# neptune-ai/open-solution-mapping-challenge

Hardware: NVIDIA H100
Metric: 300x300 tiles/sec fwd+bwd ResNet101-UNet (higher is better)
Workload: dtype bf16

## Files before the change

### include/mcb200.h

```cpp
#ifndef MCB200_H_
#define MCB200_H_

#include <stddef.h>
#include <stdint.h>

#ifdef __cplusplus
extern "C" {
#endif

#define MCB_OK 0
#define MCB_ERR_INVALID (-1)
#define MCB_ERR_CUDA (-2)
#define MCB_ERR_UNSUPPORTED (-3)

const char* mcb_last_error(void);
int mcb_version(void);
int mcb_zero_bytes(void* p, size_t bytes, void* stream);


typedef struct {
  const void* x[2];
  int cin[2];
  int n, h, w;
  const void* weight;
// ... 44 lines not shown
typedef struct {
  const void* x;
  int n, h, w, cin;
  const void* weight;
  int cout;
  const float* bias;
  int relu;
  void* y;
  int ksize;
} mcb_convt_fwd_args;
int mcb_convt_fwd(const mcb_convt_fwd_args* a, void* stream);

typedef struct {
  const void* dy;
  int n, h, w, cin;
  const void* weight;
  int cout;
  void* dx;
  const void* relu_mask;
  int accumulate;
  float* dx_channel_sum;
  int ksize;
} mcb_convt_dgrad_args;
int mcb_convt_dgrad(const mcb_convt_dgrad_args* a, void* stream);

typedef struct {
  const void* dy;
  const void* x;
  int n, h, w, cin, cout;
  float* dw;
  int ksize;
} mcb_convt_wgrad_args;
int mcb_convt_wgrad(const mcb_convt_wgrad_args* a, void* stream);


int mcb_nchw_f32_to_nhwc_bf16(const float* x, void* y, int n, int c, int h, int w, void* stream);
int mcb_nhwc_bf16_to_nchw_f32(const void* x, float* y, int n, int c, int h, int w, void* stream);

int mcb_stem_im2col(const float* x_nchw, void* col, int n, int h, int w, void* stream);
int mcb_stem_pack_weight(const float* w, void* w_packed, void* stream);
int mcb_stem_unpack_wgrad(const float* dw_packed, float* dw, void* stream);

int mcb_vgg_input_im2col(const float* x_nchw, void* col, int n, int h, int w, void* stream);
int mcb_vgg_input_pack_weight(const float* w, void* w_packed, void* stream);
int mcb_vgg_input_unpack_wgrad(const float* dw_packed, float* dw, void* stream);

int mcb_bn_finalize(const float* stats, long count, const float* gamma, const float* beta, float* running_mean,
                    float* running_var, float momentum, float eps, float* scale, float* shift, float* mean,
                    float* invstd, int c, void* stream);
int mcb_bn_eval_params(const float* gamma, const float* beta, const float* running_mean, const float* running_var,
                       float eps, float* scale, float* shift, int c, void* stream);
int mcb_bn_apply(const void* z, const float* scale, const float* shift, const void* residual, const float* res_scale,
                 const float* res_shift, int relu, void* y, long pixels, int c, void* stream);
typedef struct {
  const float* stats;
  const float* gamma;
  const float* beta;
  float* running_mean;
  float* running_var;
  float* mean;
  float* invstd;
} mcb_bn_train;
int mcb_bn_train_apply(const void* z, const mcb_bn_train* bn, const void* residual, const mcb_bn_train* res_bn, int relu,
                       void* y, long pixels, int c, float momentum, float eps, void* stream);
int mcb_bn_train_apply_global(const void* z, const mcb_bn_train* bn, const void* residual, const mcb_bn_train* res_bn,
                              int relu, void* y, long pixels, long stat_count, int c, float momentum, float eps,
// ... 164 lines not shown
```

### open-solution-mapping-challenge_b200/_lib.py

```python
import ctypes as C
import os

_HERE = os.path.dirname(os.path.abspath(__file__))
LIB_PATH = os.path.join(_HERE, "libmcb200.so")

if not os.path.exists(LIB_PATH):
    raise ImportError(
        "libmcb200.so not built: run `python __graft_entry__.py` (nvcc, sm_90a). There is no CPU fallback.")

lib = C.CDLL(LIB_PATH)
lib.mcb_last_error.restype = C.c_char_p
lib.mcb_version.restype = C.c_int

vp, ci, fp = C.c_void_p, C.c_int, C.POINTER(C.c_float)


class ConvFwdArgs(C.Structure):
    _fields_ = [("x", vp * 2), ("cin", ci * 2), ("n", ci), ("h", ci), ("w", ci), ("weight", vp), ("cout", ci),
                ("ksize", ci), ("stride", ci), ("bias", vp), ("relu", ci), ("stats", vp), ("y", vp), ("scale", vp),
                ("residual", vp)]


class ConvDgradArgs(C.Structure):
    _fields_ = [("dy", vp), ("n", ci), ("h", ci), ("w", ci), ("weight", vp), ("cout", ci), ("cin_total", ci),
                ("ci_off", ci), ("cin", ci), ("ksize", ci), ("stride", ci), ("dx", vp), ("relu_mask", vp),
                ("accumulate", ci), ("bn_z", vp), ("bn_mean", vp), ("bn_invstd", vp), ("bn_dbeta", vp),
                ("bn_dgamma", vp), ("bn_gamma", vp), ("bn_beta", vp), ("dx_channel_sum", vp)]


class ConvWgradArgs(C.Structure):
    _fields_ = [("dy", vp), ("x", vp), ("n", ci), ("h", ci), ("w", ci), ("cout", ci), ("cin_total", ci),
                ("ci_off", ci), ("cin", ci), ("ksize", ci), ("stride", ci), ("dw", vp)]


class ConvtFwdArgs(C.Structure):
    _fields_ = [("x", vp), ("n", ci), ("h", ci), ("w", ci), ("cin", ci), ("weight", vp), ("cout", ci), ("bias", vp),
                ("relu", ci), ("y", vp), ("ksize", ci)]


class ConvtDgradArgs(C.Structure):
    _fields_ = [("dy", vp), ("n", ci), ("h", ci), ("w", ci), ("cin", ci), ("weight", vp), ("cout", ci), ("dx", vp),
                ("relu_mask", vp), ("accumulate", ci), ("dx_channel_sum", vp), ("ksize", ci)]


class ConvtWgradArgs(C.Structure):
    _fields_ = [("dy", vp), ("x", vp), ("n", ci), ("h", ci), ("w", ci), ("cin", ci), ("cout", ci), ("dw", vp),
                ("ksize", ci)]


def check(rc, what=""):
    if rc != 0:
        raise RuntimeError("libmcb200 %s failed (%d): %s" % (what, rc, lib.mcb_last_error().decode()))


def ptr(t):
    return None if t is None else C.c_void_p(t.data_ptr())


def stream_ptr():
    import torch
    return C.c_void_p(torch.cuda.current_stream().cuda_stream)


def call(name, args=None, *extra):
    fn = getattr(lib, name)
    if args is None:
        rc = fn(*extra, stream_ptr())
    else:
        rc = fn(C.byref(args), *extra, stream_ptr())
    check(rc, name)


class LossArgs(C.Structure):
    _fields_ = [("logits", vp), ("target", vp), ("n", ci), ("h", ci), ("w", ci), ("mode", ci), ("w0", C.c_float),
                ("sigma", C.c_float), ("size_c", C.c_float), ("dice_weight", C.c_float), ("ce_weight", C.c_float),
                ("dice_smooth", C.c_float), ("dice_activation", ci)]


cl, cf = C.c_long, C.c_float
_SIGS = {
    "mcb_nchw_f32_to_nhwc_bf16": [vp, vp, ci, ci, ci, ci, vp],
    "mcb_nhwc_bf16_to_nchw_f32": [vp, vp, ci, ci, ci, ci, vp],
    "mcb_stem_im2col": [vp, vp, ci, ci, ci, vp],
    "mcb_stem_pack_weight": [vp, vp, vp],
    "mcb_stem_unpack_wgrad": [vp, vp, vp],
    "mcb_vgg_input_im2col": [vp, vp, ci, ci, ci, vp],
    "mcb_vgg_input_pack_weight": [vp, vp, vp],
    "mcb_vgg_input_unpack_wgrad": [vp, vp, vp],
    "mcb_maxpool2_bwd_skip_relu": [vp, vp, vp, vp, ci, ci, ci, ci, vp],
    "mcb_bn_finalize": [vp, cl, vp, vp, vp, vp, cf, cf, vp, vp, vp, vp, ci, vp],
    "mcb_bn_eval_params": [vp, vp, vp, vp, cf, vp, vp, ci, vp],
    "mcb_bn_apply": [vp, vp, vp, vp, vp, vp, ci, vp, cl, ci, vp],
    "mcb_bn_bwd_reduce": [vp, vp, vp, vp, vp, vp, vp, cl, ci, vp],
    "mcb_bn_bwd_apply": [vp, vp, vp, vp, vp, vp, vp, vp, vp, vp, ci, cl, ci, vp],
    "mcb_bn_bwd_apply_global": [vp, vp, vp, vp, vp, vp, vp, vp, vp, vp, ci, cl, cl, ci, vp],
    "mcb_channel_sum": [vp, vp, cl, ci, vp],
    "mcb_det_sum_f32": [vp, ci, cl, cl, cl, vp, cl, vp],
    "mcb_maxpool2_fwd": [vp, vp, ci, ci, ci, ci, vp],
    "mcb_maxpool2_bwd": [vp, vp, vp, ci, ci, ci, ci, ci, vp],
    "mcb_final_conv_fwd": [vp, vp, vp, vp, ci, ci, ci, ci, ci, vp],
    "mcb_final_conv_bwd": [vp, vp, vp, vp, vp, vp, ci, ci, ci, ci, ci, vp],
    "mcb_adam_step": [vp, vp, vp, vp, vp, cl, cf, C.c_double, C.c_double, cf, cf, ci, cf, vp],
    "mcb_adam_step_dyn": [vp, vp, vp, vp, vp, cl, vp, cf, cf, cf, cf, cf, vp],
    "mcb_cast_f32_bf16": [vp, vp, cl, vp],
    "mcb_loss_partials": [C.POINTER(LossArgs), vp, vp],
    "mcb_loss_grad": [C.POINTER(LossArgs), vp, cl, cf, vp, vp, vp],
    "mcb_softmax2": [vp, vp, ci, ci, ci, vp],
}
for _n, _a in _SIGS.items():
    getattr(lib, _n).argtypes = _a
    getattr(lib, _n).restype = ci
for _n in ("mcb_conv_fwd", "mcb_conv_dgrad", "mcb_conv_wgrad", "mcb_convt_fwd", "mcb_convt_dgrad", "mcb_convt_wgrad"):
    getattr(lib, _n).restype = ci


def dp(t):
    return None if t is None else t.data_ptr()


def fcall(name, *args):
    import torch
    rc = getattr(lib, name)(*args, torch.cuda.current_stream().cuda_stream)
    check(rc, name)

_SIGS2 = {
    "mcb_resize_bilinear_f64": [vp, vp, vp, ci, ci, ci, ci, ci, ci, vp],
    "mcb_threshold_layers": [vp, ci, vp, vp, vp, ci, ci, ci, ci, ci, vp],
    "mcb_ccl_label": [vp, ci, vp, vp, vp, ci, ci, ci, vp],
    "mcb_morph_rect": [vp, vp, ci, ci, ci, ci, ci, ci, vp],
    "mcb_add_dropped_objects": [vp, vp, vp, vp, ci, ci, ci, vp],
    "mcb_instance_scores": [vp, vp, ci, vp, vp, vp, vp, ci, ci, ci, ci, vp],
}
for _n, _a in _SIGS2.items():
    getattr(lib, _n).argtypes = _a
    getattr(lib, _n).restype = ci

_SIGS3 = {
    "mcb_crf_rgb_from_normalized": [vp, vp, ci, ci, ci, vp],
    "mcb_dense_crf": [vp, vp, vp, vp, ci, ci, ci, cf, cf, cf, cf, cf, ci, vp],
}
for _n, _a in _SIGS3.items():
    getattr(lib, _n).argtypes = _a
    getattr(lib, _n).restype = ci

lib.mcb_watershed.argtypes = [vp, ci, vp, vp, vp, vp, ci, ci, ci, ci, vp]
lib.mcb_watershed.restype = ci
# ... 94 lines not shown
```

### open-solution-mapping-challenge_b200/csrc/conv_gemm.cu

```cuda
#include "host_common.h"
#include "conv_gemm.cuh"
#include "../../include/mcb200.h"
#include <algorithm>
#include <mutex>
#include <stdlib.h>

namespace mcb {

static void pick_tile(int Wv, int Hv, int N, int max_rows, int row_mult, int* pbw, int* pbh, int* pbn) {
  double best = -1.0;
  int bbw = 1, bbh = 1, bbn = 1;
  for (int bw = 1; bw <= std::min(max_rows, std::min(Wv, 256)); ++bw) {
    for (int bh = 1; bw * bh <= max_rows && bh <= std::min(Hv, 256); ++bh) {
      const int bn_max = std::min(256, max_rows / (bw * bh));
      for (int bn = 1; bn <= bn_max; ++bn) {
        if (bn > N && row_mult == 1) break;
        const int rows = bw * bh * bn;
        if (rows % row_mult != 0) continue;
        const long tiles = (long)((Wv + bw - 1) / bw) * ((Hv + bh - 1) / bh) * ((N + bn - 1) / bn);
        const double eff = (double)Wv * Hv * N / ((double)tiles * max_rows);
        const double score = eff + 1e-6 * bw + 1e-9 * bh;
        if (score > best) {
          best = score;
          bbw = bw; bbh = bh; bbn = bn;
        }
      }
    }
  }
  *pbw = bbw; *pbh = bbh; *pbn = bbn;
}

constexpr int kSmemBudget = 227 * 1024;
constexpr int kMaxStagesHalo = 9, kMaxStages = 6;
constexpr int kWgradMaxStages = 8;
constexpr int kTwoStagingMinStages = 3;
constexpr int kHaloMinChannels = 128;
constexpr int kBn256MinWaveX10 = 6;
constexpr int kWgradWavesX10 = 10;
constexpr int kWgradMinKb = 6;
constexpr int kWgradKbTarget = 64;
constexpr int kWgradMinWaveX10 = 4;

static_assert(conv_smem(32, 32, true, kMaxStagesHalo, 1, 0).fits && conv_smem(32, 32, false, kMaxStages, 1, 0).fits &&
                  wgrad_smem(32, kWgradMaxStages).fits, "the mbarriers outgrow their reserve at the deepest rings");

struct TestHooks { int force_bn, halo, wgrad_splits; };
static TestHooks test_hooks() {
  auto get = [](const char* name, int dflt) {
    const char* v = getenv(name);
    return v ? atoi(v) : dflt;
  };
  return {get("MCB_FORCE_BN", 0), get("MCB_HALO", 2), get("MCB_WGRAD_SPLITS", 0)};
}

template <auto Kernel, class Params>
static int launch_kernel(const Params& p, dim3 grid, int threads, size_t smem, cudaStream_t st) {
  static bool attr_set = false;
  if (!attr_set) {
    MCB_CHECK_CUDA(cudaFuncSetAttribute(Kernel, cudaFuncAttributeMaxDynamicSharedMemorySize, kSmemBudget));
    attr_set = true;
  }
  Kernel<<<grid, threads, smem, st>>>(p);
  MCB_LAUNCH_CHECK();
  return MCB_OK;
}

static int launch_conv_kernel(int BN, int BK, bool b_mn, bool halo, const ConvGemmParams& p, dim3 grid, size_t smem,
                              cudaStream_t st) {
  auto with_flag = [](bool v, auto f) { return v ? f(std::true_type()) : f(std::false_type()); };
  return with_flag(BK == 64, [&](auto bk64) { return with_flag(b_mn, [&](auto mn) { return with_flag(halo, [&](auto h) {
    constexpr int K = decltype(bk64)::value ? 64 : 32;
    constexpr bool M = decltype(mn)::value, H = decltype(h)::value;
    switch (BN) {
      case 256: return launch_kernel<conv_gemm_kernel<256, K, M, H>>(p, grid, kConvThreads, smem, st);
      case 128: return launch_kernel<conv_gemm_kernel<128, K, M, H>>(p, grid, kConvThreads, smem, st);
      case 64: return launch_kernel<conv_gemm_kernel<64, K, M, H>>(p, grid, kConvThreads, smem, st);
      case 32: return launch_kernel<conv_gemm_kernel<32, K, M, H>>(p, grid, kConvThreads, smem, st);
    }
    return fail(MCB_ERR_UNSUPPORTED, "unsupported BN %d", BN);
  }); }); });
}

static int launch_conv(int BN, int BK, bool b_mn, ConvGemmParams& p, int m_tiles, int n_tiles, int phases,
                       cudaStream_t st, bool halo = false) {
  auto layout = [&](int stages, int out_bufs) { return conv_smem(BN, BK, halo, stages, out_bufs, p.aux_mode != 0); };
  const int stage = layout(0, 0).stage, max_stages = halo ? kMaxStagesHalo : kMaxStages;
  p.out_bufs = (kSmemBudget - layout(0, 2).bytes) / stage >= kTwoStagingMinStages ? 2 : 1;
  p.stages = std::max(2, std::min(max_stages, (kSmemBudget - layout(0, p.out_bufs).bytes) / stage));
  p.m_tiles = m_tiles; p.n_tiles = n_tiles; p.phases = phases;
  const size_t smem = layout(p.stages, p.out_bufs).bytes;
  const long total = (long)m_tiles * n_tiles * phases;
  dim3 grid((unsigned)std::min<long>(total, num_sms()), 1, 1);
  const int nch = n_tiles * BN;
  const bool red = conv_reduces(p);
  p.red_stride = 2 * nch;
  if (red && (long)grid.x * p.red_stride > kConvRedCap)
    return fail(MCB_ERR_UNSUPPORTED, "conv: reduction rows %u x %d exceed the workspace", grid.x, p.red_stride);
  const int r = launch_conv_kernel(BN, BK, b_mn, halo, p, grid, smem, st);
  if (r || !red) return r;
  const int rows = (int)grid.x;
  if (p.aux_mode == 0) {
    conv_red_finish_kernel<<<det_finish_grid(2L * nch, rows), kDetFinishThreads, 0, st>>>(
        0L, rows, (long)p.red_stride, 2L * nch, (long)nch, p.stats + p.n_off, (long)p.stats_c);
  } else {
    conv_red_finish_kernel<<<det_finish_grid(nch, rows), kDetFinishThreads, 0, st>>>(
        0L, rows, (long)p.red_stride, (long)nch, (long)nch, p.bn_dbeta + p.n_off, 0L);
    if (p.aux_mode == 2)
      conv_red_finish_kernel<<<det_finish_grid(nch, rows), kDetFinishThreads, 0, st>>>(
          (long)nch, rows, (long)p.red_stride, (long)nch, (long)nch, p.bn_dgamma + p.n_off, 0L);
  }
  MCB_LAUNCH_CHECK();
  return MCB_OK;
}

static bool use_halo(int ksize, int stride, int W, int H, int k_channels) {
  const int mode = test_hooks().halo;
  if (ksize != 3 || stride != 1 || mode == 0) return false;
  if (mode == 2) return k_channels >= kHaloMinChannels && W % 8 == 0 && H % 16 == 0 && W >= 80;
  const double eff = (double)W * H / ((double)((W + 7) / 8) * 8 * ((H + 15) / 16) * 16);
  return eff >= 0.8;
}

static int widest_bn(int n) {
  for (int bn : {256, 128, 64})
    if (n % bn == 0) return bn;
  return 32;
}

static int pick_bn(int n_total, long m_tiles, int phases) {
  int bn = widest_bn(n_total);
  const long sms = num_sms();
// ... 54 lines not shown
}

static int plan_conv(ConvGemmParams& p, const TapRule& rule, const View* a, int nsrc, const View& out, const void* aux,
                     const void* w, int w_pitch, int w_off, bool b_mn, cudaStream_t st) {
  const bool phased = rule.scatter && rule.stride == 2, parity_a = !rule.scatter && rule.stride == 2;
  const int Wv = phased ? out.w / 2 : out.w, Hv = phased ? out.h / 2 : out.h, N = out.n;
  int BK = 64;
  for (int s = 0; s < nsrc; ++s)
    if (a[s].c % 64 != 0) BK = 32;
  const bool halo = use_halo(rule.ksize, rule.stride, Wv, Hv, nsrc == 2 ? std::min(a[0].c, a[1].c) : a[0].c);
  if (halo) { p.bw = 8; p.bh = 16; p.bn = 1; }
  else pick_tile(Wv, Hv, N, 128, 1, &p.bw, &p.bh, &p.bn);
  p.rows = p.bw * p.bh * p.bn;
  p.Wv = Wv; p.Hv = Hv; p.Nimg = N;
  p.tiles_x = (Wv + p.bw - 1) / p.bw;
  p.tiles_y = (Hv + p.bh - 1) / p.bh;
  const long m_tiles = (long)p.tiles_x * p.tiles_y * ((N + p.bn - 1) / p.bn);

  bool used[4] = {false, false, false, false};
  int phases = 0, nt = 0, phase_slot[4];
  for (int v = 0; v < (phased ? 4 : 1); ++v) {
    const int start = nt;
    for_each_tap(rule, v >> 1, v & 1, [&](int slot, int dx, int dy, int wtap) {
      for (int s = 0; s < nsrc; ++s) {
        TapDesc& t = p.taps[nt++];
        t.src = slot + s; t.dx = dx; t.dy = dy; t.nchunks = a[s].c / BK; t.wk0 = s == 0 ? 0 : a[0].c; t.wtap = wtap;
        used[slot + s] = true;
      }
    });
    if (nt == start) continue;
    p.tap_start[phases] = start; p.tap_count[phases] = nt - start;
    phase_slot[phases++] = phased ? v : -1;
  }
  for (int v = 0; v < 4; ++v)
    if (used[v])
      if (int r = encode_view(&p.tmA[v], a[parity_a ? 0 : v], parity_a ? v : -1, BK, halo ? kHaloW : p.bw,
                              halo ? kHaloH : p.bh, p.bn)) return r;

  const int BN = pick_bn(out.c, m_tiles, phases);
  const int wtaps = rule.ksize * rule.ksize;
  if (int r = b_mn ? encode_weight(&p.tmB, w, wtaps, a[0].c, w_pitch, w_off, out.c, chunk_width(BN), BK)
                   : encode_weight(&p.tmB, w, wtaps, out.c, w_pitch, 0, w_pitch, BK, BN)) return r;
  const View aux_view = {aux, out.n, out.h, out.w, out.c};
  for (int ph = 0; ph < phases; ++ph) {
    if (int r = encode_view(&p.tmD[ph], out, phase_slot[ph], chunk_width(BN), p.bw, p.bh, p.bn)) return r;
    if (aux)
      if (int r = encode_view(&p.tmX[ph], aux_view, phase_slot[ph], chunk_width(BN), p.bw, p.bh, p.bn)) return r;
  }
  return launch_conv(BN, BK, b_mn, p, (int)m_tiles, out.c / BN, phases, st, halo);
}

static long wgrad_region_offset(cudaStream_t st) {
  static std::mutex mu;
  static cudaStream_t owner[kWgradRegions];
  static unsigned long last_use[kWgradRegions];
  static unsigned long clock = 0;
  std::lock_guard<std::mutex> lock(mu);
  ++clock;
  int r = 0;
  for (int i = 0; i < kWgradRegions; ++i) {
    if (last_use[i] != 0 && owner[i] == st) { r = i; break; }
    if (last_use[i] < last_use[r]) r = i;
  }
  owner[r] = st;
  last_use[r] = clock;
  return (long)r * kWgradRegionCap;
}

static int launch_wgrad(WgradParams& p, int BN, int cin_src, cudaStream_t st) {
  const int m_tiles = (p.cout + 127) / 128;
  const int n_tiles = cin_src / BN;
  const long base = (long)m_tiles * n_tiles * p.ntaps;
// ... 138 lines not shown
extern "C" int mcb_convt_fwd(const mcb_convt_fwd_args* a, void* stream) {
  MCB_REQUIRE(a && a->x && a->weight && a->y, "convt_fwd: null pointer");
  if (int r = check_c(a->cin, "convt_fwd input")) return r;
  if (int r = check_c(a->cout, "convt_fwd output")) return r;
  const int K = convt_ksize(a->ksize);
  MCB_REQUIRE(K == 3 || K == 4, "convt_fwd: ksize %d", a->ksize);
  const View x = {a->x, a->n, a->h, a->w, a->cin};
  ConvGemmParams p;
  memset(&p, 0, sizeof(p));
  p.bias = a->bias; p.relu = a->relu;
  return plan_conv(p, {K, 1, 2, true, K == 3}, &x, 1, {a->y, a->n, 2 * a->h, 2 * a->w, a->cout}, nullptr, a->weight,
                   a->cin, 0, false, static_cast<cudaStream_t>(stream));
}

extern "C" int mcb_convt_dgrad(const mcb_convt_dgrad_args* a, void* stream) {
  MCB_REQUIRE(a && a->dy && a->weight && a->dx, "convt_dgrad: null pointer");
  MCB_REQUIRE(!(a->relu_mask && a->accumulate), "convt_dgrad: relu_mask with accumulate is ill-defined");
  if (int r = check_c(a->cin, "convt_dgrad dx")) return r;
  if (int r = check_c(a->cout, "convt_dgrad dy")) return r;
  const int K = convt_ksize(a->ksize);
  MCB_REQUIRE(K == 3 || K == 4, "convt_dgrad: ksize %d", a->ksize);
  MCB_REQUIRE(!(a->dx_channel_sum && (!a->relu_mask || a->accumulate)),
              "convt_dgrad: dx_channel_sum needs relu_mask and a complete (non-accumulated) gradient");
  const View dy = {a->dy, a->n, 2 * a->h, 2 * a->w, a->cout};
  ConvGemmParams p;
  memset(&p, 0, sizeof(p));
  p.accumulate = a->accumulate;
  p.aux_mode = a->relu_mask ? 1 : 0;
  p.bn_dbeta = a->dx_channel_sum;
  return plan_conv(p, {K, 1, 2}, &dy, 1, {a->dx, a->n, a->h, a->w, a->cin}, a->relu_mask, a->weight, a->cin, 0, true,
                   static_cast<cudaStream_t>(stream));
}

extern "C" int mcb_conv_wgrad(const mcb_conv_wgrad_args* a, void* stream) {
  MCB_REQUIRE(a && a->dy && a->x && a->dw, "conv_wgrad: null pointer");
  MCB_REQUIRE(a->ksize == 1 || a->ksize == 3, "conv_wgrad: ksize %d", a->ksize);
  MCB_REQUIRE(a->stride == 1 || a->stride == 2, "conv_wgrad: stride %d", a->stride);
  if (int r = check_c(a->cout, "conv_wgrad dy")) return r;
  if (int r = check_c(a->cin, "conv_wgrad x")) return r;
  MCB_REQUIRE(a->cout % 128 == 0 || a->cout == 64 || a->cout == 32, "conv_wgrad: cout %d", a->cout);
  MCB_REQUIRE(a->stride == 1 || (a->h % 2 == 0 && a->w % 2 == 0), "conv_wgrad: stride 2 needs even H, W");
  WgradParams p;
  memset(&p, 0, sizeof(p));
  p.dw = a->dw; p.cout = a->cout; p.cin_total = a->cin_total; p.ci_off = a->ci_off;
  const View dy = {a->dy, a->n, a->h / a->stride, a->w / a->stride, a->cout}, x = {a->x, a->n, a->h, a->w, a->cin};
  return plan_wgrad(p, {a->ksize, a->ksize / 2, a->stride}, dy, x, false, static_cast<cudaStream_t>(stream));
}

extern "C" int mcb_convt_wgrad(const mcb_convt_wgrad_args* a, void* stream) {
  MCB_REQUIRE(a && a->dy && a->x && a->dw, "convt_wgrad: null pointer");
  if (int r = check_c(a->cout, "convt_wgrad dy")) return r;
  if (int r = check_c(a->cin, "convt_wgrad x")) return r;
  MCB_REQUIRE(a->cout % 128 == 0 || a->cout == 64 || a->cout == 32, "convt_wgrad: cout %d", a->cout);
  const int K = convt_ksize(a->ksize);
  MCB_REQUIRE(K == 3 || K == 4, "convt_wgrad: ksize %d", a->ksize);
  WgradParams p;
  memset(&p, 0, sizeof(p));
  p.dw = a->dw; p.cout = a->cout; p.cin_total = a->cin; p.ci_off = 0;
  const View dy = {a->dy, a->n, 2 * a->h, 2 * a->w, a->cout}, x = {a->x, a->n, a->h, a->w, a->cin};
  return plan_wgrad(p, {K, 1, 2}, dy, x, true, static_cast<cudaStream_t>(stream));
}
```

### open-solution-mapping-challenge_b200/csrc/conv_gemm.cuh

```cuda
#pragma once
#include "tc.cuh"
#include "detsum.cuh"
#include "nanmax.cuh"

namespace mcb {

constexpr int kMaxTaps = 24;

constexpr long kConvRedCap = 256L * 4096;
constexpr int kWgradRegions = 4;
constexpr long kWgradRegionCap = 4L * 1024 * 1024;
MCB_DET_WORKSPACE(float, g_conv_red, kConvRedCap, conv_red_finish_kernel)
MCB_DET_WORKSPACE(float, g_wgrad_red, kWgradRegions * kWgradRegionCap, wgrad_red_finish_kernel)
constexpr int kGemmThreads = 384;
constexpr int kProducerRegs = 40, kMmaRegs = 232;

struct TapDesc {
  int16_t src;
  int16_t dx, dy;
  int16_t nchunks;
  int32_t wk0;
  int32_t wtap;
};

// ... 52 lines not shown
  int a_chunks;
  int cin_src;
  long slice;
  long ws_off;
};

__device__ __forceinline__ uint8_t* align_up_1024(uint8_t* p) {
  const uint32_t a = static_cast<uint32_t>(__cvta_generic_to_shared(p));
  return p + ((1024u - (a & 1023u)) & 1023u);
}


constexpr int kConvThreads = 512;
constexpr int kConvProducerRegs = 24, kConvEpilogueRegs = 120, kConvMmaRegs = 184;

constexpr int kHaloW = 10, kHaloH = 18;

constexpr int kStatBytes = 4 * 8 * 16 * 4;

__host__ __device__ constexpr int chunk_width(int bn) { return bn >= 64 ? 64 : 32; }

__host__ __device__ __forceinline__ bool conv_reduces(const ConvGemmParams& p) {
  return p.stats != nullptr || p.aux_mode == 2 || (p.aux_mode == 1 && p.bn_dbeta != nullptr);
}

constexpr int kSmemAlignSlack = 1024, kConvBarrierReserve = 1536, kWgradBarrierReserve = 512;

struct ConvSmem { int a_tile, stage, a_ring, out_stage, aux_stage, stat_scratch, bars, row_ok, bytes; bool fits; };
__host__ __device__ constexpr ConvSmem conv_smem(int bn, int bk, bool halo, int stages, int out_bufs, bool aux) {
  ConvSmem l{};
  l.a_tile = halo ? (kHaloW * kHaloH * bk * 2 + 1023) / 1024 * 1024 : 128 * bk * 2;
  l.stage = (halo ? 0 : l.a_tile) + bn * bk * 2;
  l.a_ring = stages * l.stage;
  l.out_stage = l.a_ring + (halo ? 2 * l.a_tile : 0);
  l.aux_stage = l.out_stage + out_bufs * 128 * bn * 2;
  l.stat_scratch = l.aux_stage + (aux ? 2 * 128 * chunk_width(bn) * 2 : 0);
  l.bars = l.stat_scratch + kStatBytes;
  l.row_ok = l.bars + (2 * stages + 10) * 8;
  l.bytes = kSmemAlignSlack + l.bars + kConvBarrierReserve;
  l.fits = l.row_ok + 128 * 4 <= l.bars + kConvBarrierReserve;
  return l;
}

struct WgradSmem { int stage, bars, bytes; bool fits; };
__host__ __device__ constexpr WgradSmem wgrad_smem(int bn, int stages) {
  const int stage = 2 * 64 * 128 + 64 * bn * 2, bars = stages * stage;
  return {stage, bars, kSmemAlignSlack + bars + kWgradBarrierReserve, 2 * stages * 8 <= kWgradBarrierReserve};
}

struct ConvTile { int phase, nt, ncol0, x0, y0, n0; };
template <int BN>
__device__ __forceinline__ ConvTile conv_tile(const ConvGemmParams& p, int t) {
  const int mt = (t / p.phases) % p.m_tiles, nt = t / (p.phases * p.m_tiles);
  const int tx = mt % p.tiles_x, ty = (mt / p.tiles_x) % p.tiles_y, tn = mt / (p.tiles_x * p.tiles_y);
  return {t % p.phases, nt, nt * BN, tx * p.bw, ty * p.bh, tn * p.bn};
}

__device__ __forceinline__ void epi_wg_sync() { asm volatile("bar.sync 1, 128;" ::: "memory"); }

template <int BN, int BK, bool B_MN, bool HALO>
__global__ void __launch_bounds__(kConvThreads, 1) conv_gemm_kernel(const __grid_constant__ ConvGemmParams p) {
  static_assert(BK == 64 || BK == 32, "BK");
  static_assert(BN == 32 || BN == 64 || BN == 128 || BN == 256, "BN");
  constexpr int A_ROW_BYTES = BK * 2;
  constexpr ConvSmem SIZES = conv_smem(BN, BK, HALO, 0, 0, false);
  constexpr int A_BYTES = SIZES.a_tile, STAGE_BYTES = SIZES.stage;
  constexpr int B_BYTES = BN * BK * 2;
  constexpr uint32_t A_LAYOUT = (BK == 64) ? tc::LAYOUT_SW128 : tc::LAYOUT_SW64;
  constexpr int CW = chunk_width(BN);
  constexpr uint32_t CW_LAYOUT = (CW == 64) ? tc::LAYOUT_SW128 : tc::LAYOUT_SW64;
  constexpr int CW_ROW_BYTES = CW * 2;
  constexpr int BMN_SUB_BYTES = BK * CW_ROW_BYTES;
  constexpr int OUT_CHUNK_BYTES = 128 * CW_ROW_BYTES;
  constexpr int OUT_CHUNKS = BN / CW;
  constexpr int OUT_TILE_BYTES = OUT_CHUNKS * OUT_CHUNK_BYTES;
  constexpr int ACC = BN / 2;

  extern __shared__ uint8_t smem_raw[];
  uint8_t* smem = align_up_1024(smem_raw);
  const int stages = p.stages;
  const int out_bufs = p.out_bufs;
  const int aux_mode = p.aux_mode;
  const ConvSmem L = conv_smem(BN, BK, HALO, stages, out_bufs, aux_mode != 0);
  uint8_t* a_ring = smem + L.a_ring;
  uint8_t* out_stage = smem + L.out_stage;
  uint8_t* aux_stage = smem + L.aux_stage;
  float* stat_scratch = reinterpret_cast<float*>(smem + L.stat_scratch);
  uint64_t* full_bar = reinterpret_cast<uint64_t*>(smem + L.bars);
  uint64_t* empty_bar = full_bar + stages;
  uint64_t* a_full_bar = empty_bar + stages;
  uint64_t* a_empty_bar = a_full_bar + 2;
  uint64_t* aux_full_bar = a_empty_bar + 2;
  uint64_t* staged_bar = aux_full_bar + 2;
  uint64_t* drained_bar = staged_bar + 2;
  int* row_ok = reinterpret_cast<int*>(smem + L.row_ok);

  const int warp = __shfl_sync(0xffffffffu, (int)(threadIdx.x >> 5), 0);
  const int lane = threadIdx.x & 31;
  const int tiles_per_phase = p.m_tiles * p.n_tiles;
  const int total_tiles = tiles_per_phase * p.phases;

  if (warp == 0 && lane == 0) {
    for (int s = 0; s < stages; ++s) {
      tc::mbar_init(&full_bar[s], 1);
      tc::mbar_init(&empty_bar[s], 2);
    }
    for (int b = 0; b < 2; ++b) {
      tc::mbar_init(&a_full_bar[b], 1);
      tc::mbar_init(&a_empty_bar[b], 2);
      tc::mbar_init(&aux_full_bar[b], 1);
      tc::mbar_init(&staged_bar[b], 8);
      tc::mbar_init(&drained_bar[b], 1);
    }
    tc::fence_barrier_init();
// ... 89 lines not shown
    };
    if (aux_mode != 0 && wtid == 0) {
      issue_aux(blockIdx.x, 0, 0);
      issue_aux(blockIdx.x, 1, 1);
    }
    float* red_row = g_conv_red + (size_t)blockIdx.x * p.red_stride;
    const int red_half = p.red_stride >> 1;
    if (do_red)
      for (int i = wtid; i < p.red_stride; i += 128) red_row[i] = 0.f;
    auto flush_reductions = [&]() {
      if (racc_nt >= 0 && wtid < CW) {
#pragma unroll
        for (int j = 0; j < OUT_CHUNKS; ++j) {
          const int ch = racc_nt * BN + j * CW + wtid;
          red_row[ch] += racc1[j];
          red_row[red_half + ch] += racc2[j];
          racc1[j] = racc2[j] = 0.f;
        }
      }
    };

    int it = 0;
    for (int t = blockIdx.x; t < total_tiles; t += gridDim.x, ++it) {
      const auto [phase_id, nt, ncol0, x0, y0, n0] = conv_tile<BN>(p, t);
      const bool tile_full = p.rows == 128 && x0 + p.bw <= p.Wv && y0 + p.bh <= p.Hv && n0 + p.bn <= p.Nimg;
      if (do_red && nt != racc_nt) {
        flush_reductions();
        racc_nt = nt;
      }
      if (pass2 && !tile_full) {
        const int wi = wtid % p.bw, hi = (wtid / p.bw) % p.bh, ni = wtid / (p.bw * p.bh);
        row_ok[wtid] = wtid < p.rows && x0 + wi < p.Wv && y0 + hi < p.Hv && n0 + ni < p.Nimg;
      }
      const int b = it % out_bufs;
      tc::mbar_wait(&staged_bar[b], (uint32_t)(it / out_bufs) & 1);
      uint8_t* obuf = out_stage + (size_t)b * OUT_TILE_BYTES;

#pragma unroll 1
      for (int chunk = 0; chunk < OUT_CHUNKS; ++chunk) {
        uint8_t* cbuf = obuf + (size_t)chunk * OUT_CHUNK_BYTES;
        const int aslot = aux_q & 1;
        if (pass2) {
          epi_wg_sync();
          const uint8_t* abuf = aux_stage + (size_t)aslot * OUT_CHUNK_BYTES;
          if (aux_mode != 0) tc::mbar_wait(&aux_full_bar[aslot], (aux_q >> 1) & 1);
          const bool bnred = aux_mode == 2;
          const int cg = wtid % CGc, rg = wtid / CGc;
          const int ch0 = p.n_off + ncol0 + chunk * CW + cg * 8;
          float s1[8], s2[8], mu[8], is[8], sc[8], sh[8];
#pragma unroll
          for (int j = 0; j < 8; ++j) s1[j] = s2[j] = mu[j] = is[j] = sc[j] = sh[j] = 0.f;
          if (bnred) {
#pragma unroll
            for (int j = 0; j < 8; ++j) {
              mu[j] = __ldg(p.bn_mean + ch0 + j);
              is[j] = __ldg(p.bn_invstd + ch0 + j);
              sc[j] = __ldg(p.bn_gamma + ch0 + j) * is[j];
              sh[j] = __ldg(p.bn_beta + ch0 + j) - mu[j] * sc[j];
            }
          }
          const uint32_t row0_off = (uint32_t)(rg * ROWSc) * CW_ROW_BYTES;
          const int swz_rg = (CW == 64) ? 0 : (rg & 1) * 2;
#pragma unroll
          for (int rr = 0; rr < ROWSc; ++rr) {
            if (!tile_full && !row_ok[rg * ROWSc + rr]) continue;
            const int unit = (CW == 64) ? (cg ^ rr) : (cg ^ (swz_rg + (rr >> 1)));
            const uint32_t off = row0_off + (uint32_t)rr * CW_ROW_BYTES + (uint32_t)unit * 16;
            const uint4 pk = *reinterpret_cast<const uint4*>(cbuf + off);
// ... 142 lines not shown
          for (int ch = 0; ch < nch; ++ch, ++ag) {
            const int as = ag & 1;
            tc::mbar_wait(&a_full_bar[as], (ag >> 1) & 1);
            const uint32_t a_base = tc::smem_u32(a_ring + (size_t)as * A_BYTES) + (uint32_t)(wg * 8 * kHaloW * A_ROW_BYTES);
            for (int tt = 0; tt < 9; ++tt, ++i) {
              const TapDesc tap = p.taps[tap_begin + tt * nsrc + sidx];
              const tc::RingPos r = ring.step(stages);
              tc::mbar_wait(&full_bar[r.slot], r.parity);
              const uint32_t sa = a_base + (uint32_t)(((1 + tap.dy) * kHaloW + (1 + tap.dx)) * A_ROW_BYTES);
              mma_block(tc::make_smem_desc(sa, 16, kHaloW * A_ROW_BYTES, A_LAYOUT),
                        b_desc(tc::smem_u32(smem + (size_t)r.slot * STAGE_BYTES)), i == 0);
              prev_s = r.slot;
              prev_as = (tt == 8) ? as : -1;
            }
          }
        }
      } else {
        int num_kb = 0;
        for (int tp = tap_begin; tp < tap_end; ++tp) num_kb += p.taps[tp].nchunks;
        for (int i = 0; i < num_kb; ++i) {
          const tc::RingPos r = ring.step(stages);
          tc::mbar_wait(&full_bar[r.slot], r.parity);
          const uint32_t sa = tc::smem_u32(smem + (size_t)r.slot * STAGE_BYTES);
          mma_block(tc::make_smem_desc(sa + (uint32_t)(wg * 64 * A_ROW_BYTES), 16, 8 * A_ROW_BYTES, A_LAYOUT),
                    b_desc(sa + A_BYTES), i == 0);
          prev_s = r.slot;
        }
      }
      tc::wgmma_wait<0>();
      tc::fence_acc(acc);
      release_prev();
    }

    const int b = it % out_bufs;
    tc::mbar_wait(&drained_bar[b], ((uint32_t)(it / out_bufs) & 1) ^ 1);
    uint8_t* obuf = out_stage + (size_t)b * OUT_TILE_BYTES;
#pragma unroll
    for (int h = 0; h < 2; ++h) {
      const int row = r_lo + 8 * h;
      const __nv_bfloat16* rrow = nullptr;
      if (p.residual != nullptr) {
        const int wi = row % p.bw, hi = (row / p.bw) % p.bh, ni = row / (p.bw * p.bh);
        const int ox = x0 + wi, oy = y0 + hi, on = n0 + ni;
        if (row < p.rows && ox < p.Wv && oy < p.Hv && on < p.Nimg) {
          const int fy = oy * p.mask_s + (p.mask_s == 2 ? (phase_id >> 1) : 0);
          const int fx = ox * p.mask_s + (p.mask_s == 2 ? (phase_id & 1) : 0);
          rrow = p.residual + (size_t)((on * p.mask_H + fy) * p.mask_W + fx) * p.mask_C + p.n_off + ncol0;
        }
      }
      uint8_t* rowp = obuf + (size_t)row * CW_ROW_BYTES;
      const int swz = (CW == 64) ? (row & 7) : ((row >> 1) & 3);
#pragma unroll
      for (int j = 0; j < BN / 8; ++j) {
        const int col = 8 * j + 2 * (lane & 3);
        float v0 = acc[4 * j + 2 * h], v1 = acc[4 * j + 2 * h + 1];
        if (p.scale != nullptr) {
          const float2 sv = __ldg(reinterpret_cast<const float2*>(p.scale + p.n_off + ncol0 + col));
          v0 *= sv.x; v1 *= sv.y;
        }
        if (p.bias != nullptr) {
          const float2 bv = __ldg(reinterpret_cast<const float2*>(p.bias + p.n_off + ncol0 + col));
          v0 += bv.x; v1 += bv.y;
        }
        if (rrow != nullptr) {
          const float2 rv = __bfloat1622float2(*reinterpret_cast<const __nv_bfloat162*>(rrow + col));
          v0 += rv.x; v1 += rv.y;
        }
        if (p.relu) { v0 = relu_nan(v0); v1 = relu_nan(v1); }
// ... 143 lines not shown
```

### open-solution-mapping-challenge_b200/ops.py

```python
import ctypes as C

import torch

from . import _lib as L


def _chk(t, dtype=torch.bfloat16):
    assert t.is_cuda and t.is_contiguous() and t.dtype == dtype, (t.device, t.is_contiguous(), t.dtype)
    return t


def pack_conv_weight(w):
    co, ci, kh, kw = w.shape
    return w.permute(2, 3, 0, 1).reshape(kh * kw, co, ci).contiguous()


def unpack_conv_weight(wp, k):
    t, co, ci = wp.shape
    return wp.reshape(k, k, co, ci).permute(2, 3, 0, 1).contiguous()


def pack_convt_weight(w):
    ci, co, kh, kw = w.shape
    return w.permute(2, 3, 1, 0).reshape(kh * kw, co, ci).contiguous()
# ... 29 lines not shown
    a.residual = _chk(residual).data_ptr() if residual is not None else None
    L.call("mcb_conv_fwd", a)
    return out


def conv_dgrad(dy, w, ksize, stride, in_hw, cin=None, ci_off=0, relu_mask=None, accumulate=False, out=None,
               bn_reduce=None, channel_sum=None):
    _chk(dy); _chk(w)
    n = dy.shape[0]
    h, wd = in_hw
    cout, cin_total = w.shape[1], w.shape[2]
    cin = cin_total if cin is None else cin
    if out is None:
        assert not accumulate
        out = torch.empty((n, h, wd, cin), dtype=torch.bfloat16, device=dy.device)
    a = L.ConvDgradArgs()
    a.dy = dy.data_ptr(); a.n, a.h, a.w = n, h, wd
    a.weight = w.data_ptr(); a.cout = cout; a.cin_total = cin_total; a.ci_off = ci_off; a.cin = cin
    a.ksize = ksize; a.stride = stride
    a.dx = _chk(out).data_ptr()
    a.relu_mask = _chk(relu_mask).data_ptr() if relu_mask is not None else None
    a.accumulate = int(accumulate)
    if bn_reduce is not None:
        z, mean, invstd, gamma, beta, dbeta, dgamma = bn_reduce
        a.bn_z = _chk(z).data_ptr(); a.bn_mean = mean.data_ptr(); a.bn_invstd = invstd.data_ptr()
        a.bn_gamma = gamma.data_ptr(); a.bn_beta = beta.data_ptr()
        a.bn_dbeta = dbeta.data_ptr(); a.bn_dgamma = dgamma.data_ptr()
    if channel_sum is not None:
        a.dx_channel_sum = _chk(channel_sum, torch.float32).data_ptr()
    L.call("mcb_conv_dgrad", a)
    return out


def conv_wgrad(dy, x, dw, ksize, stride, ci_off=0):
    _chk(dy); _chk(x); _chk(dw, torch.float32)
    n, h, wd, cin = x.shape
    a = L.ConvWgradArgs()
    a.dy = dy.data_ptr(); a.x = x.data_ptr(); a.n, a.h, a.w = n, h, wd
    a.cout = dw.shape[1]; a.cin_total = dw.shape[2]; a.ci_off = ci_off; a.cin = cin
    a.ksize = ksize; a.stride = stride; a.dw = dw.data_ptr()
    L.call("mcb_conv_wgrad", a)
    return dw


def _convt_ksize(taps):
    assert taps in (9, 16), taps
    return 3 if taps == 9 else 4


def convt_fwd(x, w, bias=None, relu=False, out=None):
    _chk(x); _chk(w)
    n, h, wd, cin = x.shape
    cout = w.shape[1]
    assert w.shape[1:] == (cout, cin), (w.shape, cin)
    if out is None:
        out = torch.empty((n, 2 * h, 2 * wd, cout), dtype=torch.bfloat16, device=x.device)
    a = L.ConvtFwdArgs()
    a.x = x.data_ptr(); a.n, a.h, a.w, a.cin = n, h, wd, cin
    a.weight = w.data_ptr(); a.cout = cout
    a.bias = _chk(bias, torch.float32).data_ptr() if bias is not None else None
    a.relu = int(relu); a.y = _chk(out).data_ptr(); a.ksize = _convt_ksize(w.shape[0])
    L.call("mcb_convt_fwd", a)
    return out


def convt_dgrad(dy, w, relu_mask=None, accumulate=False, out=None, channel_sum=None):
# ... 247 lines not shown
```

Measured before the change: 1001.

## Stage conv output in operand ring for single-wave launches; drop BK for short reductions

When a non-halo conv launch fits in a single wave, the output tile is now staged in the operand ring (out_bufs=0), with a named barrier between the MMA warpgroups. This frees shared memory for more pipeline stages. Separately, reducing convs with short K and many tiles switch from BK=64 to BK=32 so that double-buffered output staging fits. It also adds a launch-info query for introspection, and reusing the ring adds synchronisation and the risk of overwriting operands still being read.

```diff
diff --git a/include/mcb200.h b/include/mcb200.h
--- a/include/mcb200.h
+++ b/include/mcb200.h
@@ -100,6 +100,11 @@
   int ksize;
 } mcb_convt_wgrad_args;
 int mcb_convt_wgrad(const mcb_convt_wgrad_args* a, void* stream);
+
+typedef struct {
+  int bn, bk, halo, stages, out_bufs, tiles, grid, smem_bytes;
+} mcb_conv_launch_info;
+int mcb_conv_last_launch(mcb_conv_launch_info* out);
 
 
 int mcb_nchw_f32_to_nhwc_bf16(const float* x, void* y, int n, int c, int h, int w, void* stream);
diff --git a/open-solution-mapping-challenge_b200/_lib.py b/open-solution-mapping-challenge_b200/_lib.py
--- a/open-solution-mapping-challenge_b200/_lib.py
+++ b/open-solution-mapping-challenge_b200/_lib.py
@@ -46,6 +46,10 @@
 class ConvtWgradArgs(C.Structure):
     _fields_ = [("dy", vp), ("x", vp), ("n", ci), ("h", ci), ("w", ci), ("cin", ci), ("cout", ci), ("dw", vp),
                 ("ksize", ci)]
+
+
+class ConvLaunchInfo(C.Structure):
+    _fields_ = [(f, ci) for f in ("bn", "bk", "halo", "stages", "out_bufs", "tiles", "grid", "smem_bytes")]
 
 
 def check(rc, what=""):
@@ -112,6 +116,8 @@
     getattr(lib, _n).restype = ci
 for _n in ("mcb_conv_fwd", "mcb_conv_dgrad", "mcb_conv_wgrad", "mcb_convt_fwd", "mcb_convt_dgrad", "mcb_convt_wgrad"):
     getattr(lib, _n).restype = ci
+lib.mcb_conv_last_launch.argtypes = [C.POINTER(ConvLaunchInfo)]
+lib.mcb_conv_last_launch.restype = ci
 
 
 def dp(t):
diff --git a/open-solution-mapping-challenge_b200/csrc/conv_gemm.cu b/open-solution-mapping-challenge_b200/csrc/conv_gemm.cu
--- a/open-solution-mapping-challenge_b200/csrc/conv_gemm.cu
+++ b/open-solution-mapping-challenge_b200/csrc/conv_gemm.cu
@@ -34,6 +34,7 @@
 constexpr int kMaxStagesHalo = 9, kMaxStages = 6;
 constexpr int kWgradMaxStages = 8;
 constexpr int kTwoStagingMinStages = 3;
+constexpr int kShortMainLoopK = 256;
 constexpr int kHaloMinChannels = 128;
 constexpr int kBn256MinWaveX10 = 6;
 constexpr int kWgradWavesX10 = 10;
@@ -42,7 +43,24 @@
 constexpr int kWgradMinWaveX10 = 4;
 
 static_assert(conv_smem(32, 32, true, kMaxStagesHalo, 1, 0).fits && conv_smem(32, 32, false, kMaxStages, 1, 0).fits &&
-                  wgrad_smem(32, kWgradMaxStages).fits, "the mbarriers outgrow their reserve at the deepest rings");
+                  conv_smem(32, 32, false, kMaxStages, 0, 0).fits && wgrad_smem(32, kWgradMaxStages).fits,
+              "the mbarriers outgrow their reserve at the deepest rings");
+
+constexpr int conv_stages(int bn, int bk, bool halo, int out_bufs, bool aux) {
+  const int n = (kSmemBudget - conv_smem(bn, bk, halo, 0, out_bufs, aux).bytes) /
+                conv_smem(bn, bk, halo, 0, 0, aux).stage;
+  return std::max(2, std::min(halo ? kMaxStagesHalo : kMaxStages, n));
+}
+
+constexpr bool ring_holds_output_tile() {
+  const int bns[] = {32, 64, 128, 256}, bks[] = {32, 64};
+  for (int bn : bns)
+    for (int bk : bks)
+      for (bool aux : {false, true})
+        if (conv_stages(bn, bk, false, 0, aux) * conv_smem(bn, bk, false, 0, 0, aux).stage < 128 * bn * 2) return false;
+  return true;
+}
+static_assert(ring_holds_output_tile(), "an output tile staged in the operand ring overruns it");
 
 struct TestHooks { int force_bn, halo, wgrad_splits; };
 static TestHooks test_hooks() {
@@ -81,22 +99,29 @@
   }); }); });
 }
 
+static std::mutex g_last_launch_mu;
+static mcb_conv_launch_info g_last_launch{};
+
 static int launch_conv(int BN, int BK, bool b_mn, ConvGemmParams& p, int m_tiles, int n_tiles, int phases,
                        cudaStream_t st, bool halo = false) {
-  auto layout = [&](int stages, int out_bufs) { return conv_smem(BN, BK, halo, stages, out_bufs, p.aux_mode != 0); };
-  const int stage = layout(0, 0).stage, max_stages = halo ? kMaxStagesHalo : kMaxStages;
-  p.out_bufs = (kSmemBudget - layout(0, 2).bytes) / stage >= kTwoStagingMinStages ? 2 : 1;
-  p.stages = std::max(2, std::min(max_stages, (kSmemBudget - layout(0, p.out_bufs).bytes) / stage));
-  p.m_tiles = m_tiles; p.n_tiles = n_tiles; p.phases = phases;
-  const size_t smem = layout(p.stages, p.out_bufs).bytes;
+  const bool aux = p.aux_mode != 0;
   const long total = (long)m_tiles * n_tiles * phases;
   dim3 grid((unsigned)std::min<long>(total, num_sms()), 1, 1);
+  if (!halo && total <= (long)grid.x) p.out_bufs = 0;
+  else p.out_bufs = conv_stages(BN, BK, halo, 2, aux) >= kTwoStagingMinStages ? 2 : 1;
+  p.stages = conv_stages(BN, BK, halo, p.out_bufs, aux);
+  p.m_tiles = m_tiles; p.n_tiles = n_tiles; p.phases = phases;
+  const size_t smem = conv_smem(BN, BK, halo, p.stages, p.out_bufs, aux).bytes;
   const int nch = n_tiles * BN;
   const bool red = conv_reduces(p);
   p.red_stride = 2 * nch;
   if (red && (long)grid.x * p.red_stride > kConvRedCap)
     return fail(MCB_ERR_UNSUPPORTED, "conv: reduction rows %u x %d exceed the workspace", grid.x, p.red_stride);
   const int r = launch_conv_kernel(BN, BK, b_mn, halo, p, grid, smem, st);
+  {
+    std::lock_guard<std::mutex> lock(g_last_launch_mu);
+    g_last_launch = {BN, BK, halo ? 1 : 0, p.stages, p.out_bufs, (int)total, (int)grid.x, (int)smem};
+  }
   if (r || !red) return r;
   const int rows = (int)grid.x;
   if (p.aux_mode == 0) {
@@ -217,12 +242,20 @@
     p.tap_start[phases] = start; p.tap_count[phases] = nt - start;
     phase_slot[phases++] = phased ? v : -1;
   }
+  const int BN = pick_bn(out.c, m_tiles, phases);
+  int k_tile = 0;
+  for (int i = p.tap_start[0]; i < p.tap_start[0] + p.tap_count[0]; ++i) k_tile += p.taps[i].nchunks * BK;
+  if (BK == 64 && !halo && conv_reduces(p) && m_tiles * phases * (out.c / BN) > num_sms() &&
+      k_tile <= kShortMainLoopK && conv_stages(BN, 64, false, 2, aux != nullptr) < kTwoStagingMinStages &&
+      conv_stages(BN, 32, false, 2, aux != nullptr) >= kTwoStagingMinStages) {
+    BK = 32;
+    for (int i = 0; i < nt; ++i) p.taps[i].nchunks *= 2;
+  }
   for (int v = 0; v < 4; ++v)
     if (used[v])
       if (int r = encode_view(&p.tmA[v], a[parity_a ? 0 : v], parity_a ? v : -1, BK, halo ? kHaloW : p.bw,
                               halo ? kHaloH : p.bh, p.bn)) return r;
 
-  const int BN = pick_bn(out.c, m_tiles, phases);
   const int wtaps = rule.ksize * rule.ksize;
   if (int r = b_mn ? encode_weight(&p.tmB, w, wtaps, a[0].c, w_pitch, w_off, out.c, chunk_width(BN), BK)
                    : encode_weight(&p.tmB, w, wtaps, out.c, w_pitch, 0, w_pitch, BK, BN)) return r;
@@ -427,6 +460,13 @@
                    static_cast<cudaStream_t>(stream));
 }
 
+extern "C" int mcb_conv_last_launch(mcb_conv_launch_info* out) {
+  MCB_REQUIRE(out, "conv_last_launch: null pointer");
+  std::lock_guard<std::mutex> lock(g_last_launch_mu);
+  *out = g_last_launch;
+  return MCB_OK;
+}
+
 extern "C" int mcb_conv_wgrad(const mcb_conv_wgrad_args* a, void* stream) {
   MCB_REQUIRE(a && a->dy && a->x && a->dw, "conv_wgrad: null pointer");
   MCB_REQUIRE(a->ksize == 1 || a->ksize == 3, "conv_wgrad: ksize %d", a->ksize);
diff --git a/open-solution-mapping-challenge_b200/csrc/conv_gemm.cuh b/open-solution-mapping-challenge_b200/csrc/conv_gemm.cuh
--- a/open-solution-mapping-challenge_b200/csrc/conv_gemm.cuh
+++ b/open-solution-mapping-challenge_b200/csrc/conv_gemm.cuh
@@ -108,8 +108,9 @@
   l.a_tile = halo ? (kHaloW * kHaloH * bk * 2 + 1023) / 1024 * 1024 : 128 * bk * 2;
   l.stage = (halo ? 0 : l.a_tile) + bn * bk * 2;
   l.a_ring = stages * l.stage;
-  l.out_stage = l.a_ring + (halo ? 2 * l.a_tile : 0);
-  l.aux_stage = l.out_stage + out_bufs * 128 * bn * 2;
+  const int past_ring = l.a_ring + (halo ? 2 * l.a_tile : 0);
+  l.out_stage = out_bufs == 0 ? 0 : past_ring;
+  l.aux_stage = past_ring + out_bufs * 128 * bn * 2;
   l.stat_scratch = l.aux_stage + (aux ? 2 * 128 * chunk_width(bn) * 2 : 0);
   l.bars = l.stat_scratch + kStatBytes;
   l.row_ok = l.bars + (2 * stages + 10) * 8;
@@ -133,6 +134,7 @@
 }
 
 __device__ __forceinline__ void epi_wg_sync() { asm volatile("bar.sync 1, 128;" ::: "memory"); }
+__device__ __forceinline__ void mma_wgs_sync() { asm volatile("bar.sync 2, 256;" ::: "memory"); }
 
 template <int BN, int BK, bool B_MN, bool HALO>
 __global__ void __launch_bounds__(kConvThreads, 1) conv_gemm_kernel(const __grid_constant__ ConvGemmParams p) {
@@ -156,6 +158,7 @@
   uint8_t* smem = align_up_1024(smem_raw);
   const int stages = p.stages;
   const int out_bufs = p.out_bufs;
+  const int bufs = out_bufs > 0 ? out_bufs : 1;
   const int aux_mode = p.aux_mode;
   const ConvSmem L = conv_smem(BN, BK, HALO, stages, out_bufs, aux_mode != 0);
   uint8_t* a_ring = smem + L.a_ring;
@@ -311,8 +314,8 @@
         const int wi = wtid % p.bw, hi = (wtid / p.bw) % p.bh, ni = wtid / (p.bw * p.bh);
         row_ok[wtid] = wtid < p.rows && x0 + wi < p.Wv && y0 + hi < p.Hv && n0 + ni < p.Nimg;
       }
-      const int b = it % out_bufs;
-      tc::mbar_wait(&staged_bar[b], (uint32_t)(it / out_bufs) & 1);
+      const int b = it % bufs;
+      tc::mbar_wait(&staged_bar[b], (uint32_t)(it / bufs) & 1);
       uint8_t* obuf = out_stage + (size_t)b * OUT_TILE_BYTES;
 
 #pragma unroll 1
@@ -521,8 +524,11 @@
       release_prev();
     }
 
-    const int b = it % out_bufs;
-    tc::mbar_wait(&drained_bar[b], ((uint32_t)(it / out_bufs) & 1) ^ 1);
+    if (out_bufs == 0) {
+      mma_wgs_sync();
+    }
+    const int b = it % bufs;
+    tc::mbar_wait(&drained_bar[b], ((uint32_t)(it / bufs) & 1) ^ 1);
     uint8_t* obuf = out_stage + (size_t)b * OUT_TILE_BYTES;
 #pragma unroll
     for (int h = 0; h < 2; ++h) {
diff --git a/open-solution-mapping-challenge_b200/ops.py b/open-solution-mapping-challenge_b200/ops.py
--- a/open-solution-mapping-challenge_b200/ops.py
+++ b/open-solution-mapping-challenge_b200/ops.py
@@ -85,6 +85,12 @@
     return out
 
 
+def conv_last_launch():
+    info = L.ConvLaunchInfo()
+    L.check(L.lib.mcb_conv_last_launch(C.byref(info)), "mcb_conv_last_launch")
+    return {f: getattr(info, f) for f, _ in info._fields_}
+
+
 def conv_wgrad(dy, x, dw, ksize, stride, ci_off=0):
     _chk(dy); _chk(x); _chk(dw, torch.float32)
     n, h, wd, cin = x.shape
```

After: 1024, median of 6. 1.02x the previous value.
